# yongkyung-oh/Stable-Neural-SDEs

Measured on AMD Instinct MI355X. Metric: SDE solver steps/sec (batch x steps / s), forward solve, higher is better.
Workload: dtype f32; 1 GPU; K2: Neural LNSDE (io=4,no=17) NL=2 B=1024/GPU H=128 C=21 L=101 natural-spline coeffs 30% NaN, 100 Euler steps dt=1, ts=[0,100], in-kernel Philox dW; rows_per_gpu=1024, solver_steps=100, global_rows=1024, parallelism=row-shard x1, no collective in the solver, kernel=auto, prepare=every call (weight pack + time table launch inside the timed region, as r01-r04)

## Files before the change

stable-neural-sdes_amd/csrc/snsde_m4_kernel.h:

```cpp
#pragma once
#include <type_traits>

#include "snsde_mfma_kernels.h"

namespace snsde_mfma {

template <int H_, int NHID_, int KUXT_, int YIN_, int SAVE_, int ACT_ = 0, int ACC_ = 0>
struct CfgL {
    static constexpr bool ACC = ACC_ != 0;
    static constexpr bool SWISH = ACT_ != 0;
    static constexpr int H = H_, NHID = NHID_, KUXT = KUXT_;
    static constexpr bool YIN = YIN_ != 0;
    static constexpr bool SAVE = SAVE_ != 0;
    static constexpr int NW = H / 16;
    static constexpr int NT = NW * 64;
    static constexpr int WPS = NW >= 4 ? NW / 4 : 1;
    static constexpr int KUH = H / 16;
    static constexpr int LDY = ld_for(16 * KUH, 16);
    static constexpr int LDX = ld_for(16 * (KUXT > 0 ? KUXT : 1), 16);
    static constexpr int LDA = LDY;
    static constexpr int NLAYER = NHID + 2;
    static constexpr int NSAVE = NHID + 2 + (SWISH ? NHID + 1 : 0);
    static constexpr int ZSLOT = NHID + 1;
    static constexpr int PRE0 = NHID + 2;
    static constexpr int ZB = 4;
    static constexpr int ZSTASH = 4 * ZB * 64;
    static constexpr int ROWCH = 128;
    static constexpr int XI = KUXT > 0 ? (4 * 16 * KUXT + NT - 1) / NT : 1;
    static constexpr int RS = 8;
    static constexpr int ACCF = 64;
    static constexpr int LDS_FLOATS = 4 * (LDY + 2 * LDX + 2 * LDA) + (ROWCH + 3) * RS + NW * ZSTASH + ACCF;
};

template <bool NANZ>
__device__ __forceinline__ float lean_tanh(float x) {
    const float t = __builtin_amdgcn_exp2f(fabsf(x) * -2.8853900817779268f);
    float q = (1.0f - t) * __builtin_amdgcn_rcpf(1.0f + t);
    if constexpr (NANZ) q = __builtin_fmaxf(q, 0.0f);
    return __builtin_copysignf(q, x);
}

template <bool NANZ>
__device__ __forceinline__ float lean_tanh_rel(float x) {
    const float x2 = x * x;
    float p = fmaf(x2, -0.053968253968253971f, 0.13333333333333333f);
    p = fmaf(x2, p, -0.33333333333333333f);
    p = fmaf(x * x2, p, x);
    const float q = lean_tanh<NANZ>(x);
    return fabsf(x) < 0.125f ? p : q;
}

__device__ __forceinline__ float lean_swish(float x, float scale) {
    const float e = __builtin_amdgcn_exp2f(x * -1.4426950408889634f);
    return (x * scale) * __builtin_amdgcn_rcpf(1.0f + e);
}

template <int KU>
__device__ __forceinline__ void lean_load_w(float (&w)[KU * 4], const float* __restrict__ g, int wave, int lane) {
#pragma unroll
    for (int u = 0; u < KU; ++u) {
        const f32x4 v = *reinterpret_cast<const f32x4*>(g + (((size_t)wave * KU + u) * 64 + lane) * 4);
        w[4 * u] = v[0]; w[4 * u + 1] = v[1]; w[4 * u + 2] = v[2]; w[4 * u + 3] = v[3];
    }
}

__device__ __forceinline__ void lean_gload(float& dst, uint32_t voff, const float* sbase) {
    asm volatile("s_nop 4\n\tglobal_load_dword %0, %1, %2" : "=v"(dst) : "v"(voff), "s"(lean_uniform(sbase)) : "memory");
}
__device__ __forceinline__ void lean_gstore(float v, uint32_t voff, const float* sbase) {
    asm volatile("s_nop 4\n\tglobal_store_dword %1, %0, %2" :: "v"(v), "v"(voff), "s"(lean_uniform(sbase)));
}
__device__ __forceinline__ void lean_gload4(float& d0, float& d1, float& d2, float& d3, uint32_t v0, uint32_t v1, uint32_t v2,
                                            uint32_t v3, const float* sbase) {
    asm volatile("s_nop 4\n\tglobal_load_dword %0, %4, %8\n\tglobal_load_dword %1, %5, %8\n\tglobal_load_dword %2, %6, %8\n\t"
                 "global_load_dword %3, %7, %8"
                 : "=&v"(d0), "=&v"(d1), "=&v"(d2), "=&v"(d3) : "v"(v0), "v"(v1), "v"(v2), "v"(v3), "s"(lean_uniform(sbase)) : "memory");
}
template <int KU> struct LeanB { f32x4 v[KU]; };
__device__ __forceinline__ void lean_read_b(uint32_t a, LeanB<1>& b) {
    asm volatile("s_mov_b64 exec, 0xffff\n\tds_read_b128 %0, %[a]\n\ts_mov_b64 exec, -1" : "=&v"(b.v[0]) : [a] "v"(a));
}
__device__ __forceinline__ void lean_read_b(uint32_t a, LeanB<2>& b) {
    asm volatile("s_mov_b64 exec, 0xffff\n\tds_read_b128 %0, %[a]\n\tds_read_b128 %1, %[a] offset:64\n\ts_mov_b64 exec, -1"
                 : "=&v"(b.v[0]), "=&v"(b.v[1]) : [a] "v"(a));
}
__device__ __forceinline__ void lean_read_b(uint32_t a, LeanB<3>& b) {
    asm volatile("s_mov_b64 exec, 0xffff\n\tds_read_b128 %0, %[a]\n\tds_read_b128 %1, %[a] offset:64\n\tds_read_b128 %2, %[a] offset:128\n\t"
                 "s_mov_b64 exec, -1" : "=&v"(b.v[0]), "=&v"(b.v[1]), "=&v"(b.v[2]) : [a] "v"(a));
}
__device__ __forceinline__ void lean_read_b(uint32_t a, LeanB<4>& b) {
    asm volatile("s_mov_b64 exec, 0xffff\n\tds_read_b128 %0, %[a]\n\tds_read_b128 %1, %[a] offset:64\n\tds_read_b128 %2, %[a] offset:128\n\t"
                 "ds_read_b128 %3, %[a] offset:192\n\ts_mov_b64 exec, -1"
                 : "=&v"(b.v[0]), "=&v"(b.v[1]), "=&v"(b.v[2]), "=&v"(b.v[3]) : [a] "v"(a));
}
__device__ __forceinline__ void lean_read_b(uint32_t a, LeanB<5>& b) {
    asm volatile("s_mov_b64 exec, 0xffff\n\tds_read_b128 %0, %[a]\n\tds_read_b128 %1, %[a] offset:64\n\tds_read_b128 %2, %[a] offset:128\n\t"
                 "ds_read_b128 %3, %[a] offset:192\n\tds_read_b128 %4, %[a] offset:256\n\ts_mov_b64 exec, -1"
                 : "=&v"(b.v[0]), "=&v"(b.v[1]), "=&v"(b.v[2]), "=&v"(b.v[3]), "=&v"(b.v[4]) : [a] "v"(a));
}
__device__ __forceinline__ void lean_read_b(uint32_t a, LeanB<6>& b) {
    asm volatile("s_mov_b64 exec, 0xffff\n\tds_read_b128 %0, %[a]\n\tds_read_b128 %1, %[a] offset:64\n\tds_read_b128 %2, %[a] offset:128\n\t"
                 "ds_read_b128 %3, %[a] offset:192\n\tds_read_b128 %4, %[a] offset:256\n\tds_read_b128 %5, %[a] offset:320\n\t"
                 "s_mov_b64 exec, -1"
                 : "=&v"(b.v[0]), "=&v"(b.v[1]), "=&v"(b.v[2]), "=&v"(b.v[3]), "=&v"(b.v[4]), "=&v"(b.v[5]) : [a] "v"(a));
}
__device__ __forceinline__ void lean_read_b(uint32_t a, LeanB<8>& b) {
    asm volatile("s_mov_b64 exec, 0xffff\n\tds_read_b128 %0, %[a]\n\tds_read_b128 %1, %[a] offset:64\n\tds_read_b128 %2, %[a] offset:128\n\t"
                 "ds_read_b128 %3, %[a] offset:192\n\tds_read_b128 %4, %[a] offset:256\n\tds_read_b128 %5, %[a] offset:320\n\t"
                 "ds_read_b128 %6, %[a] offset:384\n\tds_read_b128 %7, %[a] offset:448\n\ts_mov_b64 exec, -1"
                 : "=&v"(b.v[0]), "=&v"(b.v[1]), "=&v"(b.v[2]), "=&v"(b.v[3]), "=&v"(b.v[4]), "=&v"(b.v[5]), "=&v"(b.v[6]), "=&v"(b.v[7])
                 : [a] "v"(a));
}
__device__ __forceinline__ void lean_read_b_carried(uint32_t a, LeanB<1>& b) {
    asm volatile("s_mov_b64 exec, 0xffff\n\tds_read_b128 %0, %[a]\n\ts_mov_b64 exec, -1" : "+v"(b.v[0]) : [a] "v"(a));
}
__device__ __forceinline__ void lean_read_b_carried(uint32_t a, LeanB<2>& b) {
    asm volatile("s_mov_b64 exec, 0xffff\n\tds_read_b128 %0, %[a]\n\tds_read_b128 %1, %[a] offset:64\n\ts_mov_b64 exec, -1"
                 : "+v"(b.v[0]), "+v"(b.v[1]) : [a] "v"(a));
}
__device__ __forceinline__ void lean_read_b_carried(uint32_t a, LeanB<3>& b) {
    asm volatile("s_mov_b64 exec, 0xffff\n\tds_read_b128 %0, %[a]\n\tds_read_b128 %1, %[a] offset:64\n\tds_read_b128 %2, %[a] offset:128\n\t"
                 "s_mov_b64 exec, -1" : "+v"(b.v[0]), "+v"(b.v[1]), "+v"(b.v[2]) : [a] "v"(a));
}
__device__ __forceinline__ void lean_read_b_carried(uint32_t a, LeanB<4>& b) {
    asm volatile("s_mov_b64 exec, 0xffff\n\tds_read_b128 %0, %[a]\n\tds_read_b128 %1, %[a] offset:64\n\tds_read_b128 %2, %[a] offset:128\n\t"
                 "ds_read_b128 %3, %[a] offset:192\n\ts_mov_b64 exec, -1"
                 : "+v"(b.v[0]), "+v"(b.v[1]), "+v"(b.v[2]), "+v"(b.v[3]) : [a] "v"(a));
}
__device__ __forceinline__ void lean_read_b_carried(uint32_t a, LeanB<5>& b) {
    asm volatile("s_mov_b64 exec, 0xffff\n\tds_read_b128 %0, %[a]\n\tds_read_b128 %1, %[a] offset:64\n\tds_read_b128 %2, %[a] offset:128\n\t"
                 "ds_read_b128 %3, %[a] offset:192\n\tds_read_b128 %4, %[a] offset:256\n\ts_mov_b64 exec, -1"
                 : "+v"(b.v[0]), "+v"(b.v[1]), "+v"(b.v[2]), "+v"(b.v[3]), "+v"(b.v[4]) : [a] "v"(a));
}
__device__ __forceinline__ void lean_read_b_carried(uint32_t a, LeanB<6>& b) {
    asm volatile("s_mov_b64 exec, 0xffff\n\tds_read_b128 %0, %[a]\n\tds_read_b128 %1, %[a] offset:64\n\tds_read_b128 %2, %[a] offset:128\n\t"
                 "ds_read_b128 %3, %[a] offset:192\n\tds_read_b128 %4, %[a] offset:256\n\tds_read_b128 %5, %[a] offset:320\n\t"
                 "s_mov_b64 exec, -1"
                 : "+v"(b.v[0]), "+v"(b.v[1]), "+v"(b.v[2]), "+v"(b.v[3]), "+v"(b.v[4]), "+v"(b.v[5]) : [a] "v"(a));
}
__device__ __forceinline__ void lean_read_b_carried(uint32_t a, LeanB<8>& b) {
    asm volatile("s_mov_b64 exec, 0xffff\n\tds_read_b128 %0, %[a]\n\tds_read_b128 %1, %[a] offset:64\n\tds_read_b128 %2, %[a] offset:128\n\t"
                 "ds_read_b128 %3, %[a] offset:192\n\tds_read_b128 %4, %[a] offset:256\n\tds_read_b128 %5, %[a] offset:320\n\t"
                 "ds_read_b128 %6, %[a] offset:384\n\tds_read_b128 %7, %[a] offset:448\n\ts_mov_b64 exec, -1"
                 : "+v"(b.v[0]), "+v"(b.v[1]), "+v"(b.v[2]), "+v"(b.v[3]), "+v"(b.v[4]), "+v"(b.v[5]), "+v"(b.v[6]), "+v"(b.v[7])
                 : [a] "v"(a));
}
#undef SNSDE_RD
template <int CNT> __device__ __forceinline__ void lean_wait2(f32x4& x, f32x4& y) {
    asm volatile("s_waitcnt lgkmcnt(%2)" : "+v"(x), "+v"(y) : "n"(CNT < 15 ? CNT : 15));
}
template <int CNT> __device__ __forceinline__ void lean_wait1(f32x4& x) {
    asm volatile("s_waitcnt lgkmcnt(%1)" : "+v"(x) : "n"(CNT < 15 ? CNT : 15));
}
template <int Y, int KU, int U>
__device__ __forceinline__ void lean_gemm_from(const float (&w)[KU * 4], LeanB<KU>& b, f32x4& c, f32x4& d) {
    if constexpr (U < KU) {
        if constexpr (U + 1 < KU) lean_wait2<Y + KU - 2 - U>(b.v[U], b.v[U + 1]);
        else lean_wait1<Y>(b.v[U]);
#pragma unroll
        for (int uu = U; uu < U + 2 && uu < KU; ++uu) {
            c = __builtin_amdgcn_mfma_f32_4x4x1f32(w[4 * uu], b.v[uu][0], c, 0, 0, 4);
            d = __builtin_amdgcn_mfma_f32_4x4x1f32(w[4 * uu + 1], b.v[uu][1], d, 0, 0, 4);
            c = __builtin_amdgcn_mfma_f32_4x4x1f32(w[4 * uu + 2], b.v[uu][2], c, 0, 0, 4);
            d = __builtin_amdgcn_mfma_f32_4x4x1f32(w[4 * uu + 3], b.v[uu][3], d, 0, 0, 4);
        }
        __builtin_amdgcn_sched_barrier(0);
        lean_gemm_from<Y, KU, U + 2>(w, b, c, d);
    }
}
template <int Y, int KU>
__device__ __forceinline__ void lean_gemm(const float (&w)[KU * 4], LeanB<KU>& b, f32x4& c, f32x4& d) {
    lean_gemm_from<Y, KU, 0>(w, b, c, d);
}

typedef short s16x4 __attribute__((ext_vector_type(4)));
typedef __bf16 bf16x4 __attribute__((ext_vector_type(4)));
template <class CF> struct CfgBf16 : CF { static constexpr bool BF = true; };
template <class CF, class = void> struct lean_bf : std::false_type {};
template <class CF> struct lean_bf<CF, std::void_t<decltype(CF::BF)>> : std::bool_constant<CF::BF> {};
template <int KU> struct LeanBh { s16x4 v[KU]; };
template <bool BF, int KU> using LeanWt = std::conditional_t<BF, s16x4[KU], float[KU * 4]>;
template <bool BF, int KU> using LeanBt = std::conditional_t<BF, LeanBh<KU>, LeanB<KU>>;
template <bool BF> using LeanOp = std::conditional_t<BF, __bf16, float>;

__device__ __forceinline__ s16x4 lean_bf16x4(f32x4 v) {
    const bf16x4 b = {(__bf16)v[0], (__bf16)v[1], (__bf16)v[2], (__bf16)v[3]};
    return __builtin_bit_cast(s16x4, b);
}
template <int KU>
__device__ __forceinline__ void lean_load_w(s16x4 (&w)[KU], const float* __restrict__ g, int wave, int lane) {
#pragma unroll
    for (int u = 0; u < KU; ++u) w[u] = lean_bf16x4(*reinterpret_cast<const f32x4*>(g + (((size_t)wave * KU + u) * 64 + lane) * 4));
}
template <bool BF>
__device__ __forceinline__ uint32_t lean_op_addr(const float* buf, int roff, int col) {
    if constexpr (BF) return lean_lds_addr(buf) + (uint32_t)((roff + col) * 2);
    else return lean_lds_addr(buf + roff + col);
}
#define LEAN_RB(i, o) "\n\tds_read_b64 %" #i ", %[a] offset:" #o
#define LEAN_RB_PRE "s_mov_b64 exec, 0xffff"
#define LEAN_RB_POST "\n\ts_mov_b64 exec, -1"
__device__ __forceinline__ void lean_read_b(uint32_t a, LeanBh<1>& b) {
    asm volatile(LEAN_RB_PRE LEAN_RB(0, 0) LEAN_RB_POST : "=&v"(b.v[0]) : [a] "v"(a));
}
__device__ __forceinline__ void lean_read_b(uint32_t a, LeanBh<2>& b) {
    asm volatile(LEAN_RB_PRE LEAN_RB(0, 0) LEAN_RB(1, 32) LEAN_RB_POST : "=&v"(b.v[0]), "=&v"(b.v[1]) : [a] "v"(a));
}
__device__ __forceinline__ void lean_read_b(uint32_t a, LeanBh<3>& b) {
    asm volatile(LEAN_RB_PRE LEAN_RB(0, 0) LEAN_RB(1, 32) LEAN_RB(2, 64) LEAN_RB_POST
                 : "=&v"(b.v[0]), "=&v"(b.v[1]), "=&v"(b.v[2]) : [a] "v"(a));
}
__device__ __forceinline__ void lean_read_b(uint32_t a, LeanBh<4>& b) {
    asm volatile(LEAN_RB_PRE LEAN_RB(0, 0) LEAN_RB(1, 32) LEAN_RB(2, 64) LEAN_RB(3, 96) LEAN_RB_POST
                 : "=&v"(b.v[0]), "=&v"(b.v[1]), "=&v"(b.v[2]), "=&v"(b.v[3]) : [a] "v"(a));
}
__device__ __forceinline__ void lean_read_b(uint32_t a, LeanBh<6>& b) {
    asm volatile(LEAN_RB_PRE LEAN_RB(0, 0) LEAN_RB(1, 32) LEAN_RB(2, 64) LEAN_RB(3, 96) LEAN_RB(4, 128) LEAN_RB(5, 160) LEAN_RB_POST
                 : "=&v"(b.v[0]), "=&v"(b.v[1]), "=&v"(b.v[2]), "=&v"(b.v[3]), "=&v"(b.v[4]), "=&v"(b.v[5]) : [a] "v"(a));
}
__device__ __forceinline__ void lean_read_b(uint32_t a, LeanBh<8>& b) {
    asm volatile(LEAN_RB_PRE LEAN_RB(0, 0) LEAN_RB(1, 32) LEAN_RB(2, 64) LEAN_RB(3, 96) LEAN_RB(4, 128) LEAN_RB(5, 160)
                 LEAN_RB(6, 192) LEAN_RB(7, 224) LEAN_RB_POST
                 : "=&v"(b.v[0]), "=&v"(b.v[1]), "=&v"(b.v[2]), "=&v"(b.v[3]), "=&v"(b.v[4]), "=&v"(b.v[5]), "=&v"(b.v[6]),
                   "=&v"(b.v[7]) : [a] "v"(a));
}
__device__ __forceinline__ void lean_read_b_carried(uint32_t a, LeanBh<1>& b) {
    asm volatile(LEAN_RB_PRE LEAN_RB(0, 0) LEAN_RB_POST : "+v"(b.v[0]) : [a] "v"(a));
}
__device__ __forceinline__ void lean_read_b_carried(uint32_t a, LeanBh<2>& b) {
    asm volatile(LEAN_RB_PRE LEAN_RB(0, 0) LEAN_RB(1, 32) LEAN_RB_POST : "+v"(b.v[0]), "+v"(b.v[1]) : [a] "v"(a));
}
__device__ __forceinline__ void lean_read_b_carried(uint32_t a, LeanBh<3>& b) {
    asm volatile(LEAN_RB_PRE LEAN_RB(0, 0) LEAN_RB(1, 32) LEAN_RB(2, 64) LEAN_RB_POST
                 : "+v"(b.v[0]), "+v"(b.v[1]), "+v"(b.v[2]) : [a] "v"(a));
}
__device__ __forceinline__ void lean_read_b_carried(uint32_t a, LeanBh<6>& b) {
    asm volatile(LEAN_RB_PRE LEAN_RB(0, 0) LEAN_RB(1, 32) LEAN_RB(2, 64) LEAN_RB(3, 96) LEAN_RB(4, 128) LEAN_RB(5, 160) LEAN_RB_POST
                 : "+v"(b.v[0]), "+v"(b.v[1]), "+v"(b.v[2]), "+v"(b.v[3]), "+v"(b.v[4]), "+v"(b.v[5]) : [a] "v"(a));
}
#undef LEAN_RB
#undef LEAN_RB_PRE
#undef LEAN_RB_POST
template <int CNT> __device__ __forceinline__ void lean_wait2(s16x4& x, s16x4& y) {
    asm volatile("s_waitcnt lgkmcnt(%2)" : "+v"(x), "+v"(y) : "n"(CNT < 15 ? CNT : 15));
}
template <int CNT> __device__ __forceinline__ void lean_wait1(s16x4& x) {
    asm volatile("s_waitcnt lgkmcnt(%1)" : "+v"(x) : "n"(CNT < 15 ? CNT : 15));
}
template <int Y, int KU, int U>
__device__ __forceinline__ void lean_gemm_from(const s16x4 (&w)[KU], LeanBh<KU>& b, f32x4& c, f32x4& d) {
    if constexpr (U < KU) {
        if constexpr (U + 1 < KU) lean_wait2<Y + KU - 2 - U>(b.v[U], b.v[U + 1]);
        else lean_wait1<Y>(b.v[U]);
        c = __builtin_amdgcn_mfma_f32_4x4x4bf16_1k(w[U], b.v[U], c, 0, 0, 4);
        if constexpr (U + 1 < KU) d = __builtin_amdgcn_mfma_f32_4x4x4bf16_1k(w[U + 1], b.v[U + 1], d, 0, 0, 4);
        __builtin_amdgcn_sched_barrier(0);
        lean_gemm_from<Y, KU, U + 2>(w, b, c, d);
    }
}
template <int Y, int KU>
__device__ __forceinline__ void lean_gemm(const s16x4 (&w)[KU], LeanBh<KU>& b, f32x4& c, f32x4& d) {
    lean_gemm_from<Y, KU, 0>(w, b, c, d);
}

template <class CF, int GEO_> struct CfgSpec : CF {
    static constexpr bool SPEC = true, SPEC_GEO = GEO_ != 0;
    static constexpr int XB = 4;
    static constexpr int LDS_FLOATS = CF::LDS_FLOATS + 4 * (XB - 2) * CF::LDX;
    static_assert(CF::XI == 1 && 4 * 16 * CF::KUXT <= 16 * CF::NW && CF::ROWCH % XB == 0, "CfgSpec: one spline entry per lane, 16 lanes per step of a batch");
};
template <class CF, class = void> struct lean_spec : std::false_type {};
template <class CF> struct lean_spec<CF, std::void_t<decltype(CF::SPEC)>> : std::bool_constant<CF::SPEC> {};
template <class CF> constexpr int lean_xslots() {
    if constexpr (lean_spec<CF>::value) return CF::XB;
    else return 2;
}
template <class CF> constexpr bool lean_spec_geo() {
    if constexpr (lean_spec<CF>::value) return CF::SPEC_GEO;
    else return false;
}

#ifdef LEAN_TRACE
#define LT_DECL unsigned long long lt[10]; uint32_t* const ltl = reinterpret_cast<uint32_t*>(lds + CF::LDS_FLOATS) + tid; \
    if constexpr (!BF) { for (int i_ = 0; i_ < 12; ++i_) ltl[i_ * NT] = 0u; }
#define LT(i) if constexpr (!BF) { asm volatile("s_memtime %0" : "=s"(lt[i])); }
#define LT_ADD(slot, i) __hip_atomic_fetch_add(ltl + (slot) * NT, (uint32_t)lt[i], __ATOMIC_RELAXED, __HIP_MEMORY_SCOPE_WORKGROUP);
#define LT_COLLECT_A if constexpr (!BF) { asm volatile("s_waitcnt lgkmcnt(0)" : "+s"(lt[0]), "+s"(lt[1]), "+s"(lt[2]), "+s"(lt[3])); \
    LT_ADD(0, 0) LT_ADD(1, 1) LT_ADD(2, 2) LT_ADD(3, 3) if (n > 0) LT_ADD(10, 0) }
#define LT_COLLECT_B if constexpr (!BF) { asm volatile("s_waitcnt lgkmcnt(0)" : "+s"(lt[4]), "+s"(lt[5]), "+s"(lt[6])); LT_ADD(4, 4) LT_ADD(5, 5) LT_ADD(6, 6) }
#define LT_COLLECT if constexpr (!BF) { asm volatile("s_waitcnt lgkmcnt(0)" : "+s"(lt[7]), "+s"(lt[8]), "+s"(lt[9])); LT_ADD(7, 7) LT_ADD(8, 8) LT_ADD(9, 9) \
    if (n + 1 < N) LT_ADD(11, 9) }
#define LT_LDS_EXTRA (12 * CF::NT * sizeof(uint32_t))
#else
#define LT_DECL
#define LT(i)
#define LT_COLLECT_A
#define LT_COLLECT_B
#define LT_COLLECT
#define LT_LDS_EXTRA 0
#endif

#ifdef LEAN_KNOCKOUT
#define LEAN_KO(SP) (SP)
#else
#define LEAN_KO(SP) false
#endif
#if (defined(LEAN_KNOCKOUT) || defined(LEAN_SPEC_WPS)) && !defined(SNSDE_DEV_SUBSET)
#error "LEAN_KNOCKOUT / LEAN_SPEC_WPS are development switches (build.py variant): never part of a product build"
#endif
#ifndef LEAN_SPEC_WPS
#define LEAN_SPEC_WPS CF::WPS
#endif

#ifndef LEAN_TANH_F
#define LEAN_TANH_F lean_tanh_rel<false>
#endif
#ifndef LEAN_TANH_G
#define LEAN_TANH_G lean_tanh_rel<true>
#endif

template <class CF>
__global__ void __launch_bounds__(CF::NT, lean_spec<CF>::value ? LEAN_SPEC_WPS : CF::WPS) snsde_m4_kernel(MfmaArgs a) {
    constexpr int H = CF::H, NT = CF::NT, NHID = CF::NHID, KUH = CF::KUH, KUXT = CF::KUXT;
    constexpr int LDY = CF::LDY, LDX = CF::LDX, LDA = CF::LDA, RS = CF::RS;
    constexpr bool YIN = CF::YIN, SAVE = CF::SAVE;
    constexpr bool BF = lean_bf<CF>::value;
    constexpr bool SP = lean_spec<CF>::value;
    static_assert(!SP || (!BF && !CF::ACC && !CF::SWISH && KUXT > 0 && 16 * KUXT + 16 <= LDX), "CfgSpec: f32 relu fields with a control path");
    using OpT = LeanOp<BF>;
    extern __shared__ __attribute__((aligned(16))) float lds[];
    float* ybuf = lds;
    constexpr int XS = lean_xslots<CF>();
    float* xbuf = ybuf + 4 * LDY;
    float* bufA = xbuf + 4 * XS * LDX;
    float* bufB = bufA + 4 * LDA;
    float* rowtab = bufB + 4 * LDA;
    float* zstash_all = rowtab + (CF::ROWCH + 3) * RS;
    float* accbuf = zstash_all + CF::NW * CF::ZSTASH;

    const int tid = threadIdx.x;
    const int lane = tid & 63;
    const int wave = __builtin_amdgcn_readfirstlane(tid >> 6);
    const int r = lane & 3, s = (lane >> 2) & 3, q = lane >> 4;
    const int fo = wave * 16 + 4 * q + s;
    const uint32_t mem = blockIdx.y;
    const int mrow0 = (int)mem * a.member_rows;
    const int row0 = mrow0 + blockIdx.x * 4;
    const float* const params = a.params + (size_t)mem * a.param_stride;
    const float* const ws = a.ws + (size_t)mem * a.ws_stride;
    const int B = a.B, C = a.C, N = a.N;
    const int row = row0 + r;
    const bool row_ok = row < B;
    const int rowc = row_ok ? row : B - 1;
    const size_t BH = (size_t)B * H;
    const size_t goff = (size_t)rowc * H + fo;
    float* zstash = zstash_all + wave * CF::ZSTASH;
    const uint32_t fo4 = (uint32_t)(fo * sizeof(float)), goff4 = (uint32_t)(goff * sizeof(float));
    const int xc = a.lean_xc;
    const bool time_on = a.lean_time != 0, geo = SP ? lean_spec_geo<CF>() : a.lean_geo != 0;
    const float act_scale = a.act == SNSDE_ACT_LIPSWISH ? 0.909f : 1.0f;
    const int f_out = SP ? (int)SNSDE_DRIFT_TANH : a.f_out;
    const bool g_raw = !SP && a.g_out == SNSDE_DIFFUSION_RAW;

    int li = 0;
    LeanWt<BF, (KUXT > 0 ? KUXT : 1)> wxt;
    LeanWt<BF, KUH> wy, wh[NHID > 0 ? NHID : 1], wo;
    if constexpr (KUXT > 0) lean_load_w<KUXT>(wxt, ws + a.w_off[li++], wave, lane);
    if constexpr (YIN) lean_load_w<KUH>(wy, ws + a.w_off[li++], wave, lane);
#pragma unroll
    for (int l = 0; l < NHID; ++l) lean_load_w<KUH>(wh[l], ws + a.w_off[li++], wave, lane);
    lean_load_w<KUH>(wo, ws + a.w_off[li++], wave, lane);
    f32x4 bfr[CF::NLAYER];
#pragma unroll
    for (int l = 0; l < CF::NLAYER; ++l)
#pragma unroll
        for (int i = 0; i < 4; ++i) bfr[l][i] = (s == 0) ? ws[a.bias_off + l * H + wave * 16 + 4 * q + i] : 0.0f;

    for (int i = tid; i < 4 * (LDY + XS * LDX + 2 * LDA); i += NT) lds[i] = 0.0f;
    auto fill_rows = [&](int base) {
        for (int i = tid; i < (CF::ROWCH + 3) * RS; i += NT) {
            const int j = i % RS;
            int rr = base + i / RS + (j == 0 ? 0 : (j == 7 ? 2 : 1));
            rr = rr < N - 1 ? rr : N - 1;
            const int src = j == 0 ? 1 : j == 1 ? 6 : j == 4 ? (a.raw_time ? 0 : 2) : j == 5 ? (a.raw_time ? 10 : 3) : j == 6 ? 4 : j == 7 ? 5 : 10;
            rowtab[i] = a.step_tab[(size_t)rr * SNSDE_STEP_STRIDE + src];
        }
    };
    fill_rows(0);
    __syncthreads();

    const float sig_theta = snsde_sigmoid(params[a.off_theta]);
    const int no = a.no;
    const bool tab = SP || a.gt_off >= 0;
    const float* gt = a.gt_ext ? a.gt_ext : ws + (tab ? a.gt_off : 0);
    const bool mul_y = SP || (no == 13 || no == 17 || no == 3 || no == 6 || no == 11);
    const bool yfun = !SP && (no >= 7 && no <= 10);
    const bool mil = !SP && a.method == SNSDE_MILSTEIN;
    const bool phx = SP || a.dW == nullptr;
    const uint32_t grow = (uint32_t)(a.row_offset + row);
    const uint64_t seed = a.seed_dev ? *a.seed_dev : a.seed;
    const int rslot = a.row_out ? a.row_out[rowc] : -1;

    float yv = a.y0[goff];
    reinterpret_cast<OpT*>(ybuf)[r * LDY + fo] = (OpT)yv;
    if (row_ok) {
        a.ys[(size_t)row * H + fo] = yv;
        if constexpr (SAVE) { if (a.traj) a.traj[(size_t)row * H + fo] = yv; }
    }

    const int xw = xc + (time_on ? 2 : 0);
    const int xquota = (4 * xw + CF::NW - 1) / CF::NW;
    float ca[CF::XI], cb[CF::XI], cc[CF::XI], cd[CF::XI];
    uint32_t cvo[CF::XI];
    int xdst[CF::XI], xkind[CF::XI];
    const size_t cstride = (size_t)(a.L - 1) * 4 * C;
    [[maybe_unused]] const int xslot = SP ? ((1 + q) & 3) * (4 * LDX) : 0;
    const uint32_t S = (uint32_t)a.samples;
    const uint32_t crow0 = (uint32_t)(row0 - mrow0);
    const uint32_t srow0 = crow0 / S, srem0 = crow0 - srow0 * S;
#pragma unroll
    for (int i = 0; i < CF::XI; ++i) {
        const int li_ = SP ? (lane & 15) : lane + 64 * i, it = wave * xquota + li_;
        const bool ok = KUXT > 0 && li_ < xquota && it < 4 * xw;
        const int rr = ok ? it / xw : 0, col = ok ? it - rr * xw : 0;
        xdst[i] = ok ? rr * LDX + col : (SP ? (lane & 3) * LDX + 16 * KUXT + (lane >> 2) : -1);
        xkind[i] = col < xc ? 0 : (col == xc ? 1 : 2);
        const int gr = row0 + rr < B ? rr : B - 1 - row0, ch = col < xc ? col : 0;
        uint32_t sr = srem0 + (uint32_t)gr, gs = 0;
#pragma unroll
        for (int k = 0; k < 3; ++k) { const bool over = sr >= S; sr -= over ? S : 0u; gs += over ? 1u : 0u; }
        cvo[i] = (uint32_t)((gs * cstride + ch) * sizeof(float));
    }
    const bool has_x = SP || (KUXT > 0 && xc > 0);
    const float* ctile = a.coeffs + (size_t)srow0 * cstride;
    const uint32_t cstep = (uint32_t)(C * sizeof(float));
    const uint32_t cidx = (uint32_t)(4 * C * sizeof(float));
    auto load_coeffs = [&](int idx) {
        if (__builtin_expect(has_x, 1)) {
            const uint32_t io = (uint32_t)idx * cidx;
#pragma unroll
            for (int i = 0; i < CF::XI; ++i)
                lean_gload4(ca[i], cb[i], cc[i], cd[i], cvo[i] + io, cvo[i] + io + cstep, cvo[i] + io + 2 * cstep,
                            cvo[i] + io + 3 * cstep, ctile);
        }
    };
    auto vm_wait = [&](float& dwn, float& gtn) {
        asm volatile("s_waitcnt vmcnt(0)" : "+v"(dwn), "+v"(gtn));
#pragma unroll
        for (int i = 0; i < CF::XI; ++i) asm volatile("" : "+v"(ca[i]), "+v"(cb[i]), "+v"(cc[i]), "+v"(cd[i]));
    };
    auto store_xt = [&](float* xb, float frac, float sn, float cs) {
        if constexpr (KUXT > 0) {
#pragma unroll
            for (int i = 0; i < CF::XI; ++i) {
                float v = 0.0f;
                if (__builtin_expect(has_x, 1)) {
                    const float x3 = cd[i] * frac;
                    float q3 = x3 * 0.333333343f;
                    q3 = fmaf(fmaf(-3.0f, q3, x3), 0.333333343f, q3);
                    v = ca[i] + (cb[i] + (0.5f * cc[i] + q3) * frac) * frac;
                }
                v = xkind[i] == 0 ? v : (xkind[i] == 1 ? sn : cs);
                if (SP || xdst[i] >= 0) reinterpret_cast<OpT*>(xb)[xdst[i]] = (OpT)v;
            }
        }
    };

    const int n0 = a.step_offset;
    auto next_dw = [&](int i, float sqh, auto first) -> float {
        if (__builtin_expect(phx, 1)) {
            const int g = n0 + i;
            const int k = (int)((uint32_t)g % (uint32_t)(4 * CF::ZB));
            if (__builtin_expect((k == 0 || first.value) && !(LEAN_KO(SP) && i > 0), 0)) {
                float zq[4 * CF::ZB];
#pragma unroll
                for (int bb = 0; bb < CF::ZB; ++bb)
                    snsde_philox_normal4(seed, grow, (uint32_t)(((g - k) >> 2) + bb), (uint32_t)fo, &zq[4 * bb]);
#pragma unroll
                for (int j = 0; j < 4 * CF::ZB; ++j) zstash[j * 64 + lane] = zq[j];
            }
            return zstash[k * 64 + lane] * sqh;
        }
        float v;
        lean_gload(v, goff4, a.dW + (size_t)i * BH);
        return v;
    };

    auto gpart = [&](float y, float gtv, float dwv, float hh) -> float {
        float g = 0.0f, draw = 0.0f;
        if (__builtin_expect(yfun, 0)) {
            float p1, p2;
            const float raw = snsde_phi(no, y, p1, p2);
            g = fast_tanh(sig_theta * snsde_nan_to_num(raw));
            draw = snsde_finite(raw) ? p1 : 0.0f;
        } else
        {
            const float raw = mul_y ? gtv * y : gtv;
            if (__builtin_expect(g_raw, 0)) {
                float yp = fmaf(raw, dwv, y);
                if (mil && mul_y) yp = fmaf(0.5f * raw * gtv, fmaf(dwv, dwv, -hh), yp);
                return yp;
            }
            g = LEAN_TANH_G(sig_theta * raw);
            draw = (mul_y && snsde_finite(raw)) ? gtv : 0.0f;
        }
        float yp = fmaf(g, dwv, y);
        if (__builtin_expect(mil, 0)) yp = fmaf(0.5f * (g * ((1.0f - g * g) * sig_theta * draw)), fmaf(dwv, dwv, -hh), yp);
        return yp;
    };

    float dw_cur, gt_cur = 0.0f;
    f32x4 qa, qb;
    {
        const float* g0 = a.step_tab;
        load_coeffs(__float_as_int(g0[5]));
        float dummy = 0.0f;
        vm_wait(dummy, gt_cur);
        store_xt(xbuf, g0[4], a.raw_time ? g0[0] : g0[2], a.raw_time ? 0.0f : g0[3]);
        dw_cur = next_dw(0, g0[6], std::true_type{});
        if (tab) lean_gload(gt_cur, fo4, gt);
        if constexpr (SP) {
            const int m = 1 + q < N - 1 ? 1 + q : N - 1;
            load_coeffs(__float_as_int(a.step_tab[(size_t)m * SNSDE_STEP_STRIDE + 5]));
        } else
        load_coeffs(__float_as_int(a.step_tab[(size_t)(N > 1 ? 1 : 0) * SNSDE_STEP_STRIDE + 5]));
        vm_wait(dw_cur, gt_cur);
        qa = *reinterpret_cast<const f32x4*>(rowtab);
        qb = *reinterpret_cast<const f32x4*>(rowtab + 4);
    }
    __syncthreads();
#ifndef LEAN_PRIO_MODE
#define LEAN_PRIO_MODE 1
#endif
    if constexpr (LEAN_PRIO_MODE == 1) { if (__builtin_amdgcn_readfirstlane(tid) >= NT / 2 && CF::NW >= 8) __builtin_amdgcn_s_setprio(1); }
    if constexpr (LEAN_PRIO_MODE == 2) { if (__builtin_amdgcn_readfirstlane(tid) < NT / 2 && CF::NW >= 8) __builtin_amdgcn_s_setprio(1); }

    const uint32_t yrow = lean_op_addr<BF>(ybuf, r * LDY, 4 * s);
    const uint32_t xrow = lean_op_addr<BF>(xbuf, r * LDX, 4 * s);
    const uint32_t arow = lean_op_addr<BF>(bufA, r * LDA, 4 * s);
    const uint32_t brow = lean_op_addr<BF>(bufB, r * LDA, 4 * s);
    OpT* const aown = reinterpret_cast<OpT*>(bufA) + r * LDA + fo;
    OpT* const bown = reinterpret_cast<OpT*>(bufB) + r * LDA + fo;
    const f32x4 zero4 = {0.f, 0.f, 0.f, 0.f};

    LeanBt<BF, (KUXT > 0 ? KUXT : 1)> bx{};
    if constexpr (KUXT > 0) lean_read_b_carried(xrow, bx);
    if constexpr (SP) {
        if constexpr (KUXT == 1) asm volatile("s_waitcnt lgkmcnt(0)" : "+v"(bx.v[0]));
        else asm volatile("s_waitcnt lgkmcnt(0)" : "+v"(bx.v[0]), "+v"(bx.v[1]));
        static_assert(KUXT <= 2, "tie every fragment of bx to the wait");
        __syncthreads();
    }
    LT_DECL
    int n = 0;
    float yold = yv;
    for (int ko = 0; ko < a.T - 1; ++ko) {
    const int n_end = __builtin_amdgcn_readfirstlane(a.out_step[ko]);
    for (; n <= n_end; ++n) {
        const int rbase = (n / CF::ROWCH) * CF::ROWCH;
        if (n > 0 && n == rbase) {
            int rb = rbase;
            asm volatile("" : "+s"(rb));
            fill_rows(rb);
            __syncthreads();
        }
        const bool more = n + 1 < N;
        [[maybe_unused]] float* act_n = nullptr;
        [[maybe_unused]] uint32_t nu = 0;
        [[maybe_unused]] uint32_t sgn = 0;
        if constexpr (SAVE) {
            nu = (uint32_t)n;
            act_n = a.act_save + uoff((int)nu, (uint32_t)CF::NSAVE * (uint32_t)BH);
        }
        LT(0)
        LeanBt<BF, KUH> by;
        if constexpr (YIN) lean_read_b(yrow, by);
        asm volatile("" : "+v"(qa), "+v"(qb));
        const float h = qa[0];
        __builtin_amdgcn_sched_barrier(0);
        f32x4 c = bfr[0], d = zero4;
        if constexpr (KUXT > 0) lean_gemm<15, KUXT>(wxt, bx, c, d);
        const float ypart = gpart(yv, gt_cur, dw_cur, h);
        if constexpr (SP) {
            if constexpr (!LEAN_KO(SP)) {
                if ((n & (CF::XB - 1)) == 0) {
                    const float* rp = rowtab + (n - rbase + q) * RS;
                    const f32x4 qk = *reinterpret_cast<const f32x4*>(rp + 4);
                    const float ik = rp[3 * RS + 7];
                    store_xt(xbuf + xslot, qk[2], qk[0], qk[1]);
                    load_coeffs(__float_as_int(ik));
                }
            }
        } else {
            store_xt(xbuf + ((n + 1) & 1) * (4 * LDX), qb[2], qb[0], qb[1]);
            load_coeffs(__float_as_int(qb[3]));
        }
        __builtin_amdgcn_sched_barrier(0);
        LT(1)
        if constexpr (YIN) lean_gemm<0, KUH>(wy, by, c, d);
        LT(2)
        {
            const float pre = m4_reduce_scatter(c + d);
            const float o = CF::SWISH ? lean_swish(pre, act_scale) : fmaxf(pre, 0.0f);
            *aown = (OpT)o;
            if constexpr (SAVE) {
                if (a.act_save && row_ok) {
                    lean_gstore(o, goff4, act_n);
                    if constexpr (CF::SWISH) lean_gstore(pre, goff4, act_n + uoff(0, 0, CF::PRE0, (uint32_t)BH));
                }
                if constexpr (!CF::SWISH) sgn = o > 0.0f ? 1u : 0u;
            }
        }
        LT(3)
        __syncthreads();
        LT_COLLECT_A
        LT(4)
        float dw_nxt = 0.0f, gt_nxt = 0.0f;
        auto prep = [&]() {
            {
                const int n1 = more ? n + 1 : n;
                dw_nxt = next_dw(n1, qa[1], std::false_type{});
                if (__builtin_expect(tab, 1)) lean_gload(gt_nxt, fo4, gt + (size_t)(uint32_t)n1 * H);
            }
        };
        uint32_t cur = arow;
#pragma unroll
        for (int l = 0; l < NHID; ++l) {
            const bool toB = (l % 2 == 0);
            LeanBt<BF, KUH> bh;
            lean_read_b(cur, bh);
            __builtin_amdgcn_sched_barrier(0);
            if (l == 0) prep();
            __builtin_amdgcn_sched_barrier(0);
            if (l == 0) { LT(5) }
            c = bfr[1 + l]; d = zero4;
            lean_gemm<0, KUH>(wh[l], bh, c, d);
            const float pre = m4_reduce_scatter(c + d);
            const float o = CF::SWISH ? lean_swish(pre, act_scale) : fmaxf(pre, 0.0f);
            *(toB ? bown : aown) = (OpT)o;
            if constexpr (SAVE) {
                if (a.act_save && row_ok) {
                    lean_gstore(o, goff4, act_n + uoff(0, 0, 1 + l, (uint32_t)BH));
                    if constexpr (CF::SWISH) lean_gstore(pre, goff4, act_n + uoff(0, 0, CF::PRE0 + 1 + l, (uint32_t)BH));
                }
                if constexpr (!CF::SWISH) sgn |= (o > 0.0f ? 1u : 0u) << (1 + l);
            }
            if (l == NHID - 1) { LT(6) }
            __syncthreads();
            if (l == NHID - 1) { LT_COLLECT_B LT(7) }
            cur = toB ? brow : arow;
        }
        {
            LeanBt<BF, KUH> bo;
            lean_read_b(cur, bo);
            __builtin_amdgcn_sched_barrier(0);
            if (NHID == 0) prep();
            __builtin_amdgcn_sched_barrier(0);
            c = bfr[NHID + 1]; d = zero4;
            lean_gemm<0, KUH>(wo, bo, c, d);
        }
        LT(8)
        vm_wait(dw_nxt, gt_nxt);
        float z = m4_reduce_scatter(c + d);
        if constexpr (SAVE) {
            if (a.act_save && row_ok) lean_gstore(CF::SWISH ? z : snsde_pack_signs(z, sgn, NHID + 1), goff4, act_n + uoff(0, 0, CF::ZSLOT, (uint32_t)BH));
        }
        if (__builtin_expect(geo, 0)) z *= fast_tanh(yv);
        float f;
        if (__builtin_expect(f_out != SNSDE_DRIFT_TANH, 0)) f = f_out == SNSDE_DRIFT_TIMES_Y ? z * yv : z;
        else f = LEAN_TANH_F(z);
        if constexpr (CF::ACC) {
            if (__builtin_expect(a.acc_col >= 0, 0)) {
                float ev = 0.0f;
                if (fo < a.acc_col) {
                    const float qv = (f - fmaf(a.acc_a, yv, a.acc_b)) * snsde_stable_inv(gt_cur);
                    ev = 0.5f * qv * qv;
                }
                ev = m4_row_sum(ev);
                if (lane < 4) accbuf[wave * 4 + lane] = ev;
                __syncthreads();
                if (fo == a.acc_col) {
                    float u = 0.0f;
                    for (int w = 0; w < CF::NW; ++w) u += accbuf[w * 4 + r];
                    f = u;
                }
            }
        }
        const float ynew = fmaf(f, h, ypart);
        yold = yv;
        yv = ynew;
        reinterpret_cast<OpT*>(ybuf)[r * LDY + fo] = (OpT)ynew;
        if constexpr (SAVE) {
            if (row_ok) {
                if (a.traj) lean_gstore(ynew, goff4, a.traj + uoff((int)nu + 1, (uint32_t)BH));
                if (a.dW_out) lean_gstore(dw_cur, goff4, a.dW_out + uoff((int)nu, (uint32_t)BH));
            }
        }
        dw_cur = dw_nxt; gt_cur = gt_nxt;
        asm volatile("ds_read_b128 %0, %2\n\tds_read_b128 %1, %2 offset:16"
                     : "+v"(qa), "+v"(qb) : "v"(lean_lds_addr(rowtab + (n + 1 - rbase) * RS)));
        if constexpr (KUXT > 0) lean_read_b_carried(xrow + ((n + 1) & (XS - 1)) * (4 * LDX * 4), bx);
        LT(9)
        __syncthreads();
        LT_COLLECT
    }
    if (row_ok) {
        const float w0 = a.out_w[2 * ko], w1 = a.out_w[2 * ko + 1];
        const float o = (w0 == 0.0f) ? yv : snsde_interp_out(w0, w1, yold, yv);
        if (!a.row_out) a.ys[(size_t)(ko + 1) * BH + goff] = o;
        else if (rslot == ko + 1) a.ys[goff] = o;
    }
    }
#ifdef LEAN_TRACE
    __syncthreads();
    if (blockIdx.x == 0 && lane == 0) {
        float* o = a.ys + (a.row_out ? 0 : (size_t)(a.T - 1) * BH);
        o[wave * 16] = (float)(uint32_t)(ltl[10 * NT] - ltl[11 * NT]);
        for (int i = 1; i < 10; ++i) o[wave * 16 + i] = (float)(uint32_t)(ltl[i * NT] - ltl[(i - 1) * NT]);
    }
#endif
}

template <class CF>
int launch_lean(const MfmaArgs& a, hipStream_t stream) {
    const size_t lds_bytes = (size_t)CF::LDS_FLOATS * sizeof(float) + LT_LDS_EXTRA;
    static SnsdeLdsAttr lds_attr;
    if (const int rc = snsde_lds_attr(reinterpret_cast<const void*>(snsde_m4_kernel<CF>), lds_bytes, lds_attr)) return rc;
    const int members = a.members > 1 ? a.members : 1;
    const int grid = ((members > 1 ? a.member_rows : a.B) + 3) / 4;
    hipLaunchKernelGGL(snsde_m4_kernel<CF>, dim3(grid, members), dim3(CF::NT), lds_bytes, stream, a);
    return hipGetLastError() == hipSuccess ? SNSDE_OK : SNSDE_ERR_LAUNCH;
}

#define SNSDE_LEAN_SPEC_LIST(X) X(128, 1, 2)
__host__ __device__ constexpr bool lean_spec_instantiated(int h, int nhid, int kuxt) {
#define SNSDE_LEAN_SPEC_HAS(H_, NH_, KX_) if (h == H_ && nhid == NH_ && kuxt == KX_) return true;
    SNSDE_LEAN_SPEC_LIST(SNSDE_LEAN_SPEC_HAS)
#undef SNSDE_LEAN_SPEC_HAS
    return false;
}

template <int H>
int dispatch_lean(const MfmaPlan& p, const MfmaArgs& a, hipStream_t st) {
    const bool save = a.act_save || a.traj || a.dW_out;
    if (p.LEAN_SPEC) {
#define SNSDE_LEAN_SPEC_CASE(H_, NH_, KX_) \
        if constexpr (H == H_) { if (p.NHID == NH_ && p.KUXT == KX_) { \
            if (p.LEAN_SPEC == 2) return save ? launch_lean<CfgSpec<CfgL<H_, NH_, KX_, 1, 1>, 1>>(a, st) \
                                              : launch_lean<CfgSpec<CfgL<H_, NH_, KX_, 1, 0>, 1>>(a, st); \
            return save ? launch_lean<CfgSpec<CfgL<H_, NH_, KX_, 1, 1>, 0>>(a, st) : launch_lean<CfgSpec<CfgL<H_, NH_, KX_, 1, 0>, 0>>(a, st); } }
        SNSDE_LEAN_SPEC_LIST(SNSDE_LEAN_SPEC_CASE)
#undef SNSDE_LEAN_SPEC_CASE
        return SNSDE_ERR_UNSUPPORTED;
    }
    if (a.acc_col >= 0) {
#ifndef SNSDE_DEV_SUBSET
#define SNSDE_LEAN_ACC(NH_) \
    if constexpr (lean_fits(H, NH_, 1, true) && lean_act_save_fits(H, NH_, 1)) { \
        if (p.NHID == NH_ && p.KUXT == 1 && p.IO != 0 && a.act == SNSDE_ACT_RELU) \
            return save ? launch_lean<CfgL<H, NH_, 1, 1, 1, 0, 1>>(a, st) : launch_lean<CfgL<H, NH_, 1, 1, 0, 0, 1>>(a, st); }
        SNSDE_LEAN_ACC(0) SNSDE_LEAN_ACC(1) SNSDE_LEAN_ACC(2) SNSDE_LEAN_ACC(3)
#undef SNSDE_LEAN_ACC
#endif
        return SNSDE_ERR_UNSUPPORTED;
    }
    if (a.act != SNSDE_ACT_RELU) {
#define SNSDE_LEAN_ACT(NH_, KX_) \
    if constexpr (lean_fits(H, NH_, KX_, true)) { \
        if (p.NHID == NH_ && p.KUXT == KX_ && p.IO != 0) { \
            if (!save) return launch_lean<CfgL<H, NH_, KX_, 1, 0, 1>>(a, st); \
            if constexpr (lean_act_save_fits(H, NH_, KX_)) return launch_lean<CfgL<H, NH_, KX_, 1, 1, 1>>(a, st); \
            else return SNSDE_ERR_UNSUPPORTED; } }
#ifndef SNSDE_DEV_SUBSET
        SNSDE_LEAN_ACT(0, 1) SNSDE_LEAN_ACT(1, 1) SNSDE_LEAN_ACT(2, 1) SNSDE_LEAN_ACT(3, 1)
        SNSDE_LEAN_ACT(0, 2) SNSDE_LEAN_ACT(1, 2) SNSDE_LEAN_ACT(2, 2) SNSDE_LEAN_ACT(3, 2)
        SNSDE_LEAN_ACT(0, 3) SNSDE_LEAN_ACT(1, 3) SNSDE_LEAN_ACT(2, 3) SNSDE_LEAN_ACT(3, 3)
#endif
#undef SNSDE_LEAN_ACT
        return SNSDE_ERR_UNSUPPORTED;
    }
#ifdef SNSDE_DEV_SUBSET
    if (p.NHID == 1 && p.KUXT == 2 && p.IO != 0)
        return save ? launch_lean<CfgL<H, 1, 2, 1, 1>>(a, st) : launch_lean<CfgL<H, 1, 2, 1, 0>>(a, st);
    if (p.NHID == 1 && p.KUXT == 1 && p.IO != 0)
        return save ? launch_lean<CfgL<H, 1, 1, 1, 1>>(a, st) : launch_lean<CfgL<H, 1, 1, 1, 0>>(a, st);
    return SNSDE_ERR_UNSUPPORTED;
#else
#define SNSDE_LEAN(NH_, KX_, Y_) \
    if constexpr (lean_fits(H, NH_, KX_, Y_ != 0)) { \
        if (p.NHID == NH_ && p.KUXT == KX_ && (p.IO != 0) == (Y_ != 0)) \
            return save ? launch_lean<CfgL<H, NH_, KX_, Y_, 1>>(a, st) : launch_lean<CfgL<H, NH_, KX_, Y_, 0>>(a, st); }
#define SNSDE_LEANS(KX_, Y_) SNSDE_LEAN(0, KX_, Y_) SNSDE_LEAN(1, KX_, Y_) SNSDE_LEAN(2, KX_, Y_) SNSDE_LEAN(3, KX_, Y_)
    SNSDE_LEANS(0, 1) SNSDE_LEANS(1, 1) SNSDE_LEANS(2, 1) SNSDE_LEANS(3, 1) SNSDE_LEANS(6, 1)
    SNSDE_LEANS(1, 0) SNSDE_LEANS(2, 0) SNSDE_LEANS(3, 0) SNSDE_LEANS(6, 0)
#undef SNSDE_LEANS
#undef SNSDE_LEAN
    return SNSDE_ERR_UNSUPPORTED;
#endif
}

int dispatch_lean_h32(const MfmaPlan& p, const MfmaArgs& a, hipStream_t st);
int dispatch_lean_h64(const MfmaPlan& p, const MfmaArgs& a, hipStream_t st);
int dispatch_lean_h128(const MfmaPlan& p, const MfmaArgs& a, hipStream_t st);
int dispatch_lean_h128_two_tile(const MfmaPlan& p, const MfmaArgs& a, hipStream_t st);
int dispatch_lean_h256(const MfmaPlan& p, const MfmaArgs& a, hipStream_t st);
int dispatch_lean_h256_two_tile(const MfmaPlan& p, const MfmaArgs& a, hipStream_t st);
int dispatch_lean_bf16_h64(const MfmaPlan& p, const MfmaArgs& a, hipStream_t st);
int dispatch_lean_bf16_h128(const MfmaPlan& p, const MfmaArgs& a, hipStream_t st);
bool m4t_instantiated(int nhid, int kuxt, bool save);
bool m4s2_instantiated(int nhid, int kuxt, bool save);

}
```

Measured before the change: 614.7 million row-steps/s.

## Use wide 128-bit LDS operand reads for hidden-layer MFMA GEMMs

Adds a LeanBW operand path that loads each layer's B fragments with ds_read_b128 (one or two per lane, offset by quad) rather than per-unit reads. The 4x4x1 MFMAs then consume them through the broadcast-block selector (4+G), so each wide read feeds four MFMA groups. This is on by default for f32 configs where KUH is divisible by 4 (H=128 qualifies). It also adds off-by-default switches for splitting the diffusion tanh and for moving the next-step carry reads earlier. The aim is fewer LDS read instructions and waits per layer, at the risk of a different lane-to-data mapping and bank-access pattern that must stay correct.

```diff
diff --git a/stable-neural-sdes_amd/csrc/snsde_m4_kernel.h b/stable-neural-sdes_amd/csrc/snsde_m4_kernel.h
--- a/stable-neural-sdes_amd/csrc/snsde_m4_kernel.h
+++ b/stable-neural-sdes_amd/csrc/snsde_m4_kernel.h
@@ -173,6 +173,37 @@
     lean_gemm_from<Y, KU, 0>(w, b, c, d);
 }
 
+template <int KW> struct LeanBW { f32x4 v[KW]; };
+__device__ __forceinline__ void lean_read_bw(uint32_t a, LeanBW<1>& b) {
+    asm volatile("ds_read_b128 %0, %[a]" : "=&v"(b.v[0]) : [a] "v"(a));
+}
+__device__ __forceinline__ void lean_read_bw(uint32_t a, LeanBW<2>& b) {
+    asm volatile("ds_read_b128 %0, %[a]\n\tds_read_b128 %1, %[a] offset:256" : "=&v"(b.v[0]), "=&v"(b.v[1]) : [a] "v"(a));
+}
+template <int G>
+__device__ __forceinline__ void lean_mfma_group(const float* w, const f32x4& b, f32x4& c, f32x4& d) {
+    c = __builtin_amdgcn_mfma_f32_4x4x1f32(w[0], b[0], c, 0, 0, 4 + G);
+    d = __builtin_amdgcn_mfma_f32_4x4x1f32(w[1], b[1], d, 0, 0, 4 + G);
+    c = __builtin_amdgcn_mfma_f32_4x4x1f32(w[2], b[2], c, 0, 0, 4 + G);
+    d = __builtin_amdgcn_mfma_f32_4x4x1f32(w[3], b[3], d, 0, 0, 4 + G);
+}
+template <int Y, int KU, int J>
+__device__ __forceinline__ void lean_gemm_from(const float (&w)[KU * 4], LeanBW<KU / 4>& b, f32x4& c, f32x4& d) {
+    if constexpr (J < KU / 4) {
+        lean_wait1<Y + KU / 4 - 1 - J>(b.v[J]);
+        lean_mfma_group<0>(w + 16 * J, b.v[J], c, d);
+        lean_mfma_group<1>(w + 16 * J + 4, b.v[J], c, d);
+        lean_mfma_group<2>(w + 16 * J + 8, b.v[J], c, d);
+        lean_mfma_group<3>(w + 16 * J + 12, b.v[J], c, d);
+        __builtin_amdgcn_sched_barrier(0);
+        lean_gemm_from<Y, KU, J + 1>(w, b, c, d);
+    }
+}
+template <int Y, int KU>
+__device__ __forceinline__ void lean_gemm(const float (&w)[KU * 4], LeanBW<KU / 4>& b, f32x4& c, f32x4& d) {
+    lean_gemm_from<Y, KU, 0>(w, b, c, d);
+}
+
 typedef short s16x4 __attribute__((ext_vector_type(4)));
 typedef __bf16 bf16x4 __attribute__((ext_vector_type(4)));
 template <class CF> struct CfgBf16 : CF { static constexpr bool BF = true; };
@@ -317,6 +348,21 @@
 #endif
 #ifndef LEAN_TANH_G
 #define LEAN_TANH_G lean_tanh_rel<true>
+#else
+#define LEAN_TANH_G_CUSTOM 1
+#endif
+
+#ifndef LEAN_GPART_MODE
+#define LEAN_GPART_MODE 0
+#endif
+#if LEAN_GPART_MODE == 1 && defined(LEAN_TANH_G_CUSTOM)
+#error "LEAN_GPART_MODE 1 splits lean_tanh_rel<true> by hand: no LEAN_TANH_G override with it"
+#endif
+#ifndef LEAN_CARRY_MODE
+#define LEAN_CARRY_MODE 0
+#endif
+#ifndef LEAN_WIDE_READS
+#define LEAN_WIDE_READS 1
 #endif
 
 template <class CF>
@@ -509,6 +555,32 @@
         return yp;
     };
 
+    [[maybe_unused]] const bool gsplit = !yfun && !g_raw;
+    [[maybe_unused]] auto gpart_head = [&](float y, float gtv, float& gx, float& gpl, float& ge) {
+        if (__builtin_expect(gsplit, 1)) {
+            const float raw = mul_y ? gtv * y : gtv;
+            gx = sig_theta * raw;
+            const float x2 = gx * gx;
+            float p = fmaf(x2, -0.053968253968253971f, 0.13333333333333333f);
+            p = fmaf(x2, p, -0.33333333333333333f);
+            gpl = fmaf(gx * x2, p, gx);
+            ge = __builtin_amdgcn_exp2f(fabsf(gx) * -2.8853900817779268f);
+        }
+    };
+    [[maybe_unused]] auto gpart_tail = [&](float y, float gtv, float dwv, float hh, float gx, float gpl, float ge) -> float {
+        if (__builtin_expect(!gsplit, 0)) return gpart(y, gtv, dwv, hh);
+        float qv = (1.0f - ge) * __builtin_amdgcn_rcpf(1.0f + ge);
+        qv = __builtin_copysignf(__builtin_fmaxf(qv, 0.0f), gx);
+        const float g = fabsf(gx) < 0.125f ? gpl : qv;
+        float yp = fmaf(g, dwv, y);
+        if (__builtin_expect(mil, 0)) {
+            const float raw = mul_y ? gtv * y : gtv;
+            const float draw = (mul_y && snsde_finite(raw)) ? gtv : 0.0f;
+            yp = fmaf(0.5f * (g * ((1.0f - g * g) * sig_theta * draw)), fmaf(dwv, dwv, -hh), yp);
+        }
+        return yp;
+    };
+
     float dw_cur, gt_cur = 0.0f;
     f32x4 qa, qb;
     {
@@ -543,6 +615,12 @@
     OpT* const bown = reinterpret_cast<OpT*>(bufB) + r * LDA + fo;
     const f32x4 zero4 = {0.f, 0.f, 0.f, 0.f};
 
+    constexpr bool WIDE = LEAN_WIDE_READS != 0 && !BF && KUH % 4 == 0;
+    using LayerB = std::conditional_t<WIDE, LeanBW<(KUH >= 4 ? KUH / 4 : 1)>, LeanBt<BF, KUH>>;
+    auto read_layer = [&](uint32_t addr, LayerB& b) {
+        if constexpr (WIDE) lean_read_bw(addr + (uint32_t)q * 64u, b);
+        else lean_read_b(addr, b);
+    };
     LeanBt<BF, (KUXT > 0 ? KUXT : 1)> bx{};
     if constexpr (KUXT > 0) lean_read_b_carried(xrow, bx);
     if constexpr (SP) {
@@ -573,14 +651,25 @@
             act_n = a.act_save + uoff((int)nu, (uint32_t)CF::NSAVE * (uint32_t)BH);
         }
         LT(0)
-        LeanBt<BF, KUH> by;
-        if constexpr (YIN) lean_read_b(yrow, by);
+        LayerB by;
+        if constexpr (YIN) read_layer(yrow, by);
         asm volatile("" : "+v"(qa), "+v"(qb));
         const float h = qa[0];
         __builtin_amdgcn_sched_barrier(0);
         f32x4 c = bfr[0], d = zero4;
         if constexpr (KUXT > 0) lean_gemm<15, KUXT>(wxt, bx, c, d);
-        const float ypart = gpart(yv, gt_cur, dw_cur, h);
+        float ypart = 0.0f;
+        [[maybe_unused]] float gx = 0.0f, gpl = 0.0f, ge = 0.0f;
+        constexpr int GPM = LEAN_GPART_MODE == 1 && NHID == 0 ? 2 : LEAN_GPART_MODE;
+        auto gp_in = [&]() { asm volatile("" : "+v"(yv), "+v"(gt_cur), "+v"(dw_cur)); };
+        if constexpr (GPM == 0) ypart = gpart(yv, gt_cur, dw_cur, h);
+        if constexpr (GPM == 3) { gp_in(); ypart = gpart(yv, gt_cur, dw_cur, h); asm volatile("" : "+v"(ypart)); }
+        auto carry = [&]() {
+            asm volatile("ds_read_b128 %0, %2\n\tds_read_b128 %1, %2 offset:16"
+                         : "+v"(qa), "+v"(qb) : "v"(lean_lds_addr(rowtab + (n + 1 - rbase) * RS)));
+            if constexpr (KUXT > 0) lean_read_b_carried(xrow + ((n + 1) & (XS - 1)) * (4 * LDX * 4), bx);
+        };
+        constexpr int YC = LEAN_CARRY_MODE == 1 ? 2 + KUXT : 0;
         if constexpr (SP) {
             if constexpr (!LEAN_KO(SP)) {
                 if ((n & (CF::XB - 1)) == 0) {
@@ -627,10 +716,13 @@
 #pragma unroll
         for (int l = 0; l < NHID; ++l) {
             const bool toB = (l % 2 == 0);
-            LeanBt<BF, KUH> bh;
-            lean_read_b(cur, bh);
+            LayerB bh;
+            read_layer(cur, bh);
             __builtin_amdgcn_sched_barrier(0);
             if (l == 0) prep();
+            if constexpr (GPM == 1) {
+                if (l == 0) { gp_in(); gpart_head(yv, gt_cur, gx, gpl, ge); asm volatile("" : "+v"(gx), "+v"(gpl), "+v"(ge)); }
+            }
             __builtin_amdgcn_sched_barrier(0);
             if (l == 0) { LT(5) }
             c = bfr[1 + l]; d = zero4;
@@ -651,13 +743,20 @@
             cur = toB ? brow : arow;
         }
         {
-            LeanBt<BF, KUH> bo;
-            lean_read_b(cur, bo);
+            LayerB bo;
+            read_layer(cur, bo);
             __builtin_amdgcn_sched_barrier(0);
             if (NHID == 0) prep();
+            if constexpr (LEAN_CARRY_MODE == 1) carry();
+            if constexpr (GPM == 2) { gp_in(); ypart = gpart(yv, gt_cur, dw_cur, h); asm volatile("" : "+v"(ypart)); }
+            if constexpr (GPM == 1) {
+                asm volatile("" : "+v"(gx), "+v"(gpl), "+v"(ge), "+v"(dw_cur));
+                ypart = gpart_tail(yv, gt_cur, dw_cur, h, gx, gpl, ge);
+                asm volatile("" : "+v"(ypart));
+            }
             __builtin_amdgcn_sched_barrier(0);
             c = bfr[NHID + 1]; d = zero4;
-            lean_gemm<0, KUH>(wo, bo, c, d);
+            lean_gemm<YC, KUH>(wo, bo, c, d);
         }
         LT(8)
         vm_wait(dw_nxt, gt_nxt);
@@ -697,9 +796,7 @@
             }
         }
         dw_cur = dw_nxt; gt_cur = gt_nxt;
-        asm volatile("ds_read_b128 %0, %2\n\tds_read_b128 %1, %2 offset:16"
-                     : "+v"(qa), "+v"(qb) : "v"(lean_lds_addr(rowtab + (n + 1 - rbase) * RS)));
-        if constexpr (KUXT > 0) lean_read_b_carried(xrow + ((n + 1) & (XS - 1)) * (4 * LDX * 4), bx);
+        if constexpr (LEAN_CARRY_MODE == 0) carry();
         LT(9)
         __syncthreads();
         LT_COLLECT
```

Result: faster. 652.5 million row-steps/s (median of 6 runs) (+6.1%).
